# genlm/genlm-backend

Measured on AMD Instinct MI355X. Metric: particles/sec + logprob-kernel HBM GB/s (% of 8 TB/s), 1024 particles gpt2, higher is better.
Workload: dtype f32

## Files before the change

### genlm-backend_amd/_lib.py

```python
import ctypes as C
import os

_HERE = os.path.dirname(os.path.abspath(__file__))
LIB_PATH = os.path.join(_HERE, "libglb_hip.so")

ABI_VERSION = 9
GLB_OK, GLB_EINVAL, GLB_EUNSUPPORTED, GLB_EHIP, GLB_ENOSPC = 0, 1, 2, 3, 4
F32, BF16, F16 = 0, 1, 2
MASK_NONE, MASK_BITS, MASK_F32, MASK_PREPARED = 0, 1, 2, 3
RNG_NONE, RNG_PHILOX, RNG_NOISE = 0, 1, 2
STEP_HW_EXP = 1
GEMM_BIAS, GEMM_BIAS_GELU_TANH = 0, 1
GEMM_FORM_LARGE, GEMM_FORM_SMALL = 1, 2


class GlbError(RuntimeError):
    def __init__(self, code, msg):
        super().__init__(f"glb error {code}: {msg}")
        self.code = code


class StepArgs(C.Structure):
    _fields_ = [
        ("struct_size", C.c_uint32),
# ... 139 lines not shown
    _fields_ = [
        ("struct_size", C.c_uint32),
        ("window", C.c_void_p), ("window_out", C.c_void_p), ("polys", C.c_void_p),
        ("n_small", C.c_int32), ("n_big", C.c_int32),
        ("vocab", C.c_int64), ("max_draw_rows", C.c_int64),
        ("n_draw", C.c_void_p),
        ("n_out_rows", C.c_int64),
        ("row_slot", C.c_void_p),
        ("out", C.c_void_p), ("out_ld", C.c_int64),
        ("workspace", C.c_void_p), ("workspace_bytes", C.c_size_t),
        ("reuse_windows", C.c_int32), ("rows_from", C.c_void_p), ("rows_from_ld", C.c_int64),
    ]


class GemmArgs(C.Structure):
    _fields_ = [
        ("struct_size", C.c_uint32),
        ("m", C.c_int64), ("n", C.c_int64), ("k", C.c_int64),
        ("a", C.c_void_p), ("lda", C.c_int64),
        ("w_split", C.c_void_p),
        ("bias", C.c_void_p),
        ("c", C.c_void_p), ("ldc", C.c_int64),
        ("epilogue", C.c_int32),
    ]


class LoraJob(C.Structure):
    _fields_ = [
        ("struct_size", C.c_uint32),
        ("w_dtype", C.c_int32), ("ab_dtype", C.c_int32), ("w_transposed", C.c_int32),
        ("n_out", C.c_int64), ("k_in", C.c_int64), ("r", C.c_int64),
        ("w", C.c_void_p), ("ldw", C.c_int64),
        ("a", C.c_void_p), ("lda", C.c_int64),
        ("b", C.c_void_p), ("ldb", C.c_int64),
        ("scale", C.c_float),
        ("out", C.c_void_p), ("ldo", C.c_int64),
    ]


class LoraRowsEntry(C.Structure):
    _fields_ = [
        ("struct_size", C.c_uint32),
        ("ab_dtype", C.c_int32),
        ("n_out", C.c_int64), ("k_in", C.c_int64), ("r", C.c_int64),
        ("a", C.c_void_p), ("lda", C.c_int64),
        ("b", C.c_void_p), ("ldb", C.c_int64),
# ... 338 lines not shown
                                  _vp]),
    "glb_trie_workspace_ex": (_sz, [_i64, _i64]),
    "glb_trie_masses": (C.c_int, [C.POINTER(TrieArgs), _vp]),
    "glb_trie_rows_workspace": (_sz, [_i64, C.POINTER(TriePlan)]),
    "glb_trie_rows": (C.c_int, [C.POINTER(TrieRowsArgs), C.POINTER(TriePlan), _vp]),
    "glb_resample_workspace": (_sz, [_i64]),
    "glb_resample_systematic": (C.c_int, [_vp, _i64, C.c_uint64, C.c_uint64, _vp, _vp, _vp, _sz, _vp]),
    "glb_mt19937_seed": (None, [C.POINTER(MT19937), C.c_uint64]),
    "glb_mt19937_exponential_f32": (C.c_int, [C.POINTER(MT19937), _vp, _i64]),
    "glb_mt19937_window": (C.c_int, [C.c_uint64, _vp]),
    "glb_mt19937_jump_polys": (C.c_int, [_i64, _i32, _i32, _vp]),
    "glb_mt19937_jump_host": (C.c_int, [_vp, _vp, _vp]),
    "glb_mt19937_rows_workspace": (_sz, [_i64, _i32]),
    "glb_mt19937_exponential_rows": (C.c_int, [C.POINTER(MtRowsArgs), _vp]),
    "glb_comm_unique_id": (C.c_int, [_vp]),
    "glb_comm_init": (C.c_int, [_vp, _i32, _i32, C.POINTER(C.c_void_p)]),
    "glb_allgather_f32": (C.c_int, [_vp, _vp, _i64, _vp, _vp]),
    "glb_comm_destroy": (C.c_int, [_vp]),
    "glb_gemm_split_bytes": (_sz, [_i64, _i64]),
    "glb_gemm_split_weights": (C.c_int, [_vp, _i64, _i64, _i64, _vp, _sz, _vp]),
    "glb_gemm_f32_split": (C.c_int, [C.POINTER(GemmArgs), _vp]),
    "glb_gemm_split_pick": (C.c_int, [_i64, _i64, _i64, C.c_int, C.POINTER(C.c_int)]),
    "glb_gemm_f32_split_form": (C.c_int, [C.POINTER(GemmArgs), C.c_int, _vp]),
    "glb_gemm_split_blocks_per_cu": (C.c_int, [C.c_int, C.POINTER(C.c_int)]),
    "glb_gemm_split_form_blocks_per_cu": (C.c_int, [C.c_int, C.c_int, C.POINTER(C.c_int)]),
    "glb_lora_merge_workspace_bytes": (_sz, [_i32]),
    "glb_lora_merge": (C.c_int, [C.POINTER(LoraJob), _i32, _vp, _sz, _vp]),
    "glb_lora_rows_table_bytes": (_sz, [_i32, _i32]),
    "glb_lora_rows_table_upload": (C.c_int, [C.POINTER(LoraRowsEntry), _i32, _i32, _vp, _sz, _vp]),
    "glb_lora_rows_workspace_bytes": (_sz, [_i64, _i32]),
    "glb_lora_rows": (C.c_int, [C.POINTER(LoraRowsArgs), _vp]),
    "glb_w4_bytes": (_sz, [_i64, _i64]),
    "glb_w4_quantize": (C.c_int, [C.POINTER(W4Args), _vp]),
    "glb_w4_dequantize": (C.c_int, [C.POINTER(W4Args), _vp]),
    "glb_w4_gemm_max_rows": (C.c_int, []),
    "glb_w4_gemm_workspace_bytes": (_sz, [_i64, _i64, _i64]),
    "glb_w4_gemm": (C.c_int, [C.POINTER(W4GemmArgs), _vp]),
    "glb_dfa_bank_init": (C.c_int, [C.POINTER(DfaArgs), _vp]),
    "glb_dfa_advance": (C.c_int, [C.POINTER(DfaArgs), _vp]),
    "glb_dfa_claim_rows": (C.c_int, [C.POINTER(DfaArgs), _vp]),
    "glb_dfa_fill_masks": (C.c_int, [C.POINTER(DfaArgs), _vp]),
    "glb_dfa_mask_ids": (C.c_int, [C.POINTER(DfaArgs), _vp]),
    "glb_dfa_bank_rows": (_i64, [_sz, _i64, _i64]),
    "glb_dfa_weight_bank_init": (C.c_int, [C.POINTER(DfaWeightArgs), _vp]),
    "glb_dfa_fill_weights": (C.c_int, [C.POINTER(DfaWeightArgs), _vp]),
    "glb_dfa_weight_bank_rows": (_i64, [_sz, _i64, _i64]),
# ... 64 lines not shown
```

### genlm-backend_amd/csrc/glb_gemm.hip

```cpp
#include <hip/hip_runtime.h>

#include <cstdint>

#include "../../include/glb.h"
#include "glb_common.hpp"

namespace {

typedef __attribute__((ext_vector_type(2))) float f32x2;
typedef __attribute__((ext_vector_type(4))) float f32x4;
typedef __attribute__((ext_vector_type(2))) __bf16 bf16x2;
typedef __attribute__((ext_vector_type(8))) __bf16 bf16x8;
typedef __attribute__((ext_vector_type(4))) uint32_t u32x4;

constexpr int BK = 32, THREADS = 256, WAVES = THREADS / 64;
constexpr int PIECE = 1024;

template <int MF_, int NF_, int BLOCKS_>
struct Geom {
  static constexpr int MF = MF_, NF = NF_, BLOCKS_PER_CU = BLOCKS_;
  static constexpr int BM = WAVES * MF * 16, BN = NF * 16;
  static constexpr int B_PIECES = NF * 3;
  static constexpr int WAVE_PIECES = B_PIECES / WAVES;
  static constexpr int STAGE_BYTES = B_PIECES * PIECE;
  static constexpr int LDS_BYTES = 2 * STAGE_BYTES;
// ... 39 lines not shown
  const int64_t t = (int64_t)blockIdx.x * blockDim.x + threadIdx.x;
  if (t >= (n / 16) * kb_count * 64) return;
  const int l = (int)(t & 63);
  const int64_t blk = t >> 6, kb = blk % kb_count, nb = blk / kb_count;
  const int64_t col = nb * 16 + (l & 15), row = kb * BK + 8 * (l >> 4);
  f32x4 x0, x1;
#pragma unroll
  for (int j = 0; j < 4; ++j) {
    x0[j] = w[(row + j) * ldw + col];
    x1[j] = w[(row + 4 + j) * ldw + col];
  }
  bf16x8 h, m, lo;
  split8(x0, x1, h, m, lo);
  u32x4 *dst = out + blk * 3 * 64 + l;
  dst[0] = __builtin_bit_cast(u32x4, h);
  dst[64] = __builtin_bit_cast(u32x4, m);
  dst[128] = __builtin_bit_cast(u32x4, lo);
}

__device__ __forceinline__ void glds16(const void *src, char *lds) {
  __builtin_amdgcn_global_load_lds(src, (__attribute__((address_space(3))) void *)lds, 16, 0, 0);
}

template <class G, bool GELU>
__global__ __launch_bounds__(THREADS, G::BLOCKS_PER_CU) void gemm_split_kernel(const float *__restrict__ a, int64_t lda,
                                                                const char *__restrict__ wsplit, const float *__restrict__ bias,
                                                                float *__restrict__ c, int64_t ldc, int m, int n, int k) {
  constexpr int MF = G::MF, NF = G::NF, BM = G::BM, BN = G::BN, WAVE_PIECES = G::WAVE_PIECES, STAGE_BYTES = G::STAGE_BYTES;
  extern __shared__ __attribute__((aligned(16))) char lds[];
  const int tid = threadIdx.x, lane = tid & 63, wave = tid >> 6;
  const int ntn = n / BN, ntm = (m + BM - 1) / BM;
  const int nwg = ntm * ntn, orig = blockIdx.x, xcd = orig & 7, q = nwg >> 3, r = nwg & 7;
  const int wgid = (xcd < r ? xcd * (q + 1) : r * (q + 1) + (xcd - r) * q) + (orig >> 3);
  const int tm = wgid / ntn, tn = wgid % ntn;
  const int m0 = tm * BM, n0 = tn * BN;
  const int kt_count = k / BK;

  const float *a_src[MF];
#pragma unroll
  for (int i = 0; i < MF; ++i) {
    int row = m0 + (MF * wave + i) * 16 + (lane & 15);
    row = row < m ? row : m - 1;
    a_src[i] = a + (int64_t)row * lda + 8 * (lane >> 4);
  }
  const char *b_src[WAVE_PIECES];
  int b_dst[WAVE_PIECES];
#pragma unroll
  for (int i = 0; i < WAVE_PIECES; ++i) {
    const int p = WAVE_PIECES * wave + i, nf = p / 3, pl = p % 3;
    const int64_t nb = n0 / 16 + nf;
// ... 41 lines not shown
      load_a(kt + 1);
      stage_b(cur ^ 1, kt + 1);
    }
#pragma unroll
    for (int nf = 0; nf < NF; ++nf) {
      const bf16x8 bh = *(const bf16x8 *)(base + (0 * NF + nf) * PIECE + lane * 16);
      const bf16x8 bm = *(const bf16x8 *)(base + (1 * NF + nf) * PIECE + lane * 16);
      const bf16x8 bl = *(const bf16x8 *)(base + (2 * NF + nf) * PIECE + lane * 16);
#pragma unroll
      for (int i = 0; i < MF; ++i) {
        f32x4 t = __builtin_amdgcn_mfma_f32_16x16x32_bf16(am[i], bm, f32x4{0.f, 0.f, 0.f, 0.f}, 0, 0, 0);
        t = __builtin_amdgcn_mfma_f32_16x16x32_bf16(al[i], bh, t, 0, 0, 0);
        t = __builtin_amdgcn_mfma_f32_16x16x32_bf16(ah[i], bl, t, 0, 0, 0);
        t = __builtin_amdgcn_mfma_f32_16x16x32_bf16(am[i], bh, t, 0, 0, 0);
        t = __builtin_amdgcn_mfma_f32_16x16x32_bf16(ah[i], bm, t, 0, 0, 0);
        t = __builtin_amdgcn_mfma_f32_16x16x32_bf16(ah[i], bh, t, 0, 0, 0);
        acc[i][nf] += t;
      }
    }
    asm volatile("s_waitcnt vmcnt(0)" ::: "memory");
    __syncthreads();
  }

#pragma unroll
  for (int nf = 0; nf < NF; ++nf) {
    const int col = n0 + nf * 16 + (lane & 15);
    const float b = bcol[nf];
#pragma unroll
    for (int i = 0; i < MF; ++i) {
      const int row0 = m0 + wave * (MF * 16) + i * 16 + 4 * (lane >> 4);
#pragma unroll
      for (int j = 0; j < 4; ++j) {
        const int row = row0 + j;
        if (row < m) {
          float v = acc[i][nf][j] + b;
          if (GELU) v = gelu_tanh(v);
          c[(int64_t)row * ldc + col] = v;
        }
      }
    }
  }
}

bool shape_supported(int64_t k, int64_t n) { return k > 0 && n > 0 && n % BN_MAX == 0 && k % 64 == 0 && k <= (1 << 20) && n <= (1 << 20); }

template <class G, bool GELU>
struct Form {
  static inline std::atomic<uint64_t> lds_done{0};
  static const void *kernel() { return (const void *)gemm_split_kernel<G, GELU>; }
  static int launch(const glb_gemm_args &g, hipStream_t stream) {
    const int64_t tiles = ((g.m + G::BM - 1) / G::BM) * (g.n / G::BN);
    if (tiles > INT32_MAX / 2 || g.m > INT32_MAX / 2) return glb::api_fail(GLB_EUNSUPPORTED, "too many rows");
    hipError_t e = glb::allow_dynamic_lds(kernel(), G::LDS_BYTES, lds_done);
    if (e != hipSuccess) return glb::api_hip_fail(e, "split GEMM LDS attribute");
    hipLaunchKernelGGL((gemm_split_kernel<G, GELU>), dim3((unsigned)tiles), dim3(THREADS), G::LDS_BYTES, stream, g.a, g.lda,
                       (const char *)g.w_split, g.bias, g.c, g.ldc, (int)g.m, (int)g.n, (int)g.k);
    e = hipGetLastError();
    if (e != hipSuccess) return glb::api_hip_fail(e, "split GEMM launch");
    return GLB_OK;
  }
  static int blocks_per_cu(int *blocks) {
    hipError_t e = glb::allow_dynamic_lds(kernel(), G::LDS_BYTES, lds_done);
    if (e != hipSuccess) return glb::api_hip_fail(e, "split GEMM LDS attribute");
    e = hipOccupancyMaxActiveBlocksPerMultiprocessor(blocks, gemm_split_kernel<G, GELU>, THREADS, G::LDS_BYTES);
    if (e != hipSuccess) return glb::api_hip_fail(e, "split GEMM occupancy query");
    return GLB_OK;
  }
};

bool form_ok(int form) { return form == GLB_GEMM_FORM_LARGE || form == GLB_GEMM_FORM_SMALL; }

hipError_t device_cus(int *n_cus) {
  static std::atomic<int> cached[64];
  int dev = 0;
  hipError_t e = hipGetDevice(&dev);
  if (e != hipSuccess) return e;
  const bool slot = dev >= 0 && dev < 64;
  if (slot && (*n_cus = cached[dev].load(std::memory_order_relaxed)) > 0) return hipSuccess;
  e = hipDeviceGetAttribute(n_cus, hipDeviceAttributeMultiprocessorCount, dev);
  if (e == hipSuccess && slot) cached[dev].store(*n_cus, std::memory_order_relaxed);
  return e;
}

constexpr int PICK_TILES_NUM = 3, PICK_TILES_DEN = 2;

}

// ... 10 lines not shown
  if (!shape_supported(k, n)) return glb::api_fail(GLB_EUNSUPPORTED, "split GEMM needs n %% 128 == 0 and k %% 64 == 0");
  if (out_bytes < glb_gemm_split_bytes(k, n) || ((uintptr_t)out) % 16)
    return glb::api_fail(GLB_ENOSPC, "split weight buffer too small or not 16-byte aligned");
  const int64_t threads = (n / 16) * (k / BK) * 64;
  hipLaunchKernelGGL(split_weights_kernel, dim3(blocks_for(threads, 256)), dim3(256), 0, (hipStream_t)stream, w, k, n, ldw,
                     (u32x4 *)out);
  const hipError_t e = hipGetLastError();
  if (e != hipSuccess) return glb::api_hip_fail(e, "split_weights launch");
  return GLB_OK;
}


int glb_gemm_split_pick(int64_t m, int64_t n, int64_t k, int n_cus, int *form) {
  if (!form) return glb::api_fail(GLB_EINVAL, "null pointer");
  if (m <= 0 || n <= 0 || k <= 0 || n_cus <= 0)
    return glb::api_fail(GLB_EINVAL, "bad shape (m %lld, n %lld, k %lld, %d CUs)", (long long)m, (long long)n, (long long)k,
                         n_cus);
  if (m > INT32_MAX || n > INT32_MAX) return *form = GLB_GEMM_FORM_LARGE, GLB_OK;
  const int64_t tiles = ((m + Large::BM - 1) / Large::BM) * ((n + Large::BN - 1) / Large::BN);
  *form = tiles * PICK_TILES_DEN < (int64_t)PICK_TILES_NUM * n_cus ? GLB_GEMM_FORM_SMALL : GLB_GEMM_FORM_LARGE;
  return GLB_OK;
}

int glb_gemm_f32_split_form(const glb_gemm_args *args, int form, void *stream) {
  if (!args) return glb::api_fail(GLB_EINVAL, "null argument block");
  if (args->struct_size != sizeof(glb_gemm_args))
    return glb::api_fail(GLB_EINVAL, "glb_gemm_args.struct_size %u != %zu (ABI mismatch)", args->struct_size,
                         sizeof(glb_gemm_args));
  if (form != 0 && !form_ok(form)) return glb::api_fail(GLB_EINVAL, "bad form %d", form);
  const glb_gemm_args &g = *args;
  if (!g.a || !g.w_split || !g.c) return glb::api_fail(GLB_EINVAL, "null pointer");
  if (g.m <= 0 || g.n <= 0 || g.k <= 0 || g.lda < g.k || g.ldc < g.n)
    return glb::api_fail(GLB_EINVAL, "bad shape (m %lld, n %lld, k %lld, lda %lld, ldc %lld)", (long long)g.m,
                         (long long)g.n, (long long)g.k, (long long)g.lda, (long long)g.ldc);
  if (g.epilogue != GLB_GEMM_BIAS && g.epilogue != GLB_GEMM_BIAS_GELU_TANH)
    return glb::api_fail(GLB_EINVAL, "bad epilogue %d", g.epilogue);
  if (!shape_supported(g.k, g.n)) return glb::api_fail(GLB_EUNSUPPORTED, "split GEMM needs n %% 128 == 0 and k %% 64 == 0");
  if (((uintptr_t)g.a) % 16 || g.lda % 4 || ((uintptr_t)g.w_split) % 16)
    return glb::api_fail(GLB_EUNSUPPORTED, "split GEMM needs A and its row pitch 16-byte aligned");
  if (form == 0) {
    int n_cus = 0;
    const hipError_t e = device_cus(&n_cus);
    if (e != hipSuccess) return glb::api_hip_fail(e, "split GEMM CU count");
    const int rc = glb_gemm_split_pick(g.m, g.n, g.k, n_cus, &form);
    if (rc != GLB_OK) return rc;
  }
  const bool gelu = g.epilogue == GLB_GEMM_BIAS_GELU_TANH;
  hipStream_t s = (hipStream_t)stream;
  if (form == GLB_GEMM_FORM_SMALL) return gelu ? Form<Small, true>::launch(g, s) : Form<Small, false>::launch(g, s);
  return gelu ? Form<Large, true>::launch(g, s) : Form<Large, false>::launch(g, s);
}

int glb_gemm_f32_split(const glb_gemm_args *args, void *stream) { return glb_gemm_f32_split_form(args, 0, stream); }

int glb_gemm_split_form_blocks_per_cu(int form, int gelu, int *blocks) {
  if (!blocks) return glb::api_fail(GLB_EINVAL, "null pointer");
  if (!form_ok(form)) return glb::api_fail(GLB_EINVAL, "bad form %d", form);
  if (form == GLB_GEMM_FORM_SMALL) return gelu ? Form<Small, true>::blocks_per_cu(blocks) : Form<Small, false>::blocks_per_cu(blocks);
  return gelu ? Form<Large, true>::blocks_per_cu(blocks) : Form<Large, false>::blocks_per_cu(blocks);
}

int glb_gemm_split_blocks_per_cu(int gelu, int *blocks) {
  return glb_gemm_split_form_blocks_per_cu(GLB_GEMM_FORM_LARGE, gelu, blocks);
}

}
```

### genlm-backend_amd/engine.py

```python
import ctypes as C

import numpy as np
import torch

from . import _lib
from ._lib import GLB_EHIP, GlbError
from ._lib import (F32, BF16, F16, MASK_NONE, MASK_BITS, MASK_F32, MASK_PREPARED, RNG_NONE, RNG_PHILOX, RNG_NOISE,
                   STEP_HW_EXP, KvPlanArgs, KvPlanChunkArgs, MtRowsArgs, StepArgs, TrieArgs, TriePlan, TrieRowsArgs, MT19937, MT_POLY_WORDS, check)

_DT = {torch.float32: F32, torch.bfloat16: BF16, torch.float16: F16}


def _ptr(t):
    return None if t is None else C.c_void_p(t.data_ptr())


class LoraRowsTable:

    def __init__(self, dev, n_slots, n_modules, r_max, keep):
        self.dev, self.n_slots, self.n_modules, self.r_max, self.keep = dev, n_slots, n_modules, r_max, keep


class HostRng:

# ... 725 lines not shown
                check(self.lib.glb_gemm_split_blocks_per_cu(int(bool(gelu)), C.byref(blocks)))
            else:
                check(self.lib.glb_gemm_split_form_blocks_per_cu(int(form), int(bool(gelu)), C.byref(blocks)))
        return blocks.value

    def gemm_split_pick(self, m, n, k, n_cus=None):
        if n_cus is None:
            n_cus = torch.cuda.get_device_properties(self.device).multi_processor_count
        form = C.c_int(0)
        check(self.lib.glb_gemm_split_pick(m, n, k, n_cus, C.byref(form)))
        return form.value

    def gemm_split_weights(self, w):
        k, n = w.shape
        nbytes = self.lib.glb_gemm_split_bytes(k, n)
        if nbytes == 0 or w.dtype != torch.float32 or w.stride(1) != 1:
            return None
        if w.device != self.device:
            raise ValueError(f"tensor on {w.device}, engine on {self.device}")
        out =torch.empty(nbytes, dtype=torch.uint8, device=self.device)
        check(self.lib.glb_gemm_split_weights(_ptr(w), k, n, w.stride(0), _ptr(out), nbytes, self._stream()))
        return out

    def gemm_split(self, x, w_split, n, bias=None, gelu=False, out=None, form=None):
        k = x.shape[-1]
        x2 = x.reshape(-1, k)
        m = x2.shape[0]
        if m == 0 or x2.stride(1) != 1:
            return None
        if bias is not None:
            if bias.device != self.device:
                raise ValueError(f"bias on {bias.device}, engine on {self.device}")
            if bias.dim() != 1 or bias.numel() != n:
                raise ValueError(f"bias of shape {tuple(bias.shape)}, expected ({n},)")
            if bias.dtype != torch.float32 or bias.stride(0) != 1:
                return None
        if out is None:
            out = torch.empty((m, n), dtype=torch.float32, device=self.device)
        else:
            if out.device != self.device:
                raise ValueError(f"out on {out.device}, engine on {self.device}")
            if out.dtype != torch.float32 or tuple(out.shape) != (m, n):
                raise ValueError(f"out is {out.dtype} {tuple(out.shape)}, expected torch.float32 {(m, n)}")
            if out.stride(1) != 1 or (m > 1 and out.stride(0) < n):
                raise ValueError(f"out has strides {out.stride()}: rows of unit inner stride, at least {n} apart, are needed")
        a = _lib.GemmArgs()
        a.struct_size = C.sizeof(_lib.GemmArgs)
        a.m, a.n, a.k = m, n, k
        a.a, a.lda = x2.data_ptr(), x2.stride(0)
        a.w_split = w_split.data_ptr()
        a.bias = bias.data_ptr() if bias is not None else None
        a.c, a.ldc = out.data_ptr(), max(out.stride(0), n)
        a.epilogue = _lib.GEMM_BIAS_GELU_TANH if gelu else _lib.GEMM_BIAS
        if form is None:
            rc = self.lib.glb_gemm_f32_split(C.byref(a), self._stream())
        else:
            rc = self.lib.glb_gemm_f32_split_form(C.byref(a), int(form), self._stream())
        if rc == _lib.GLB_EUNSUPPORTED:
            return None
        check(rc)
        return out.view(*x.shape[:-1], n)

    def lora_merge(self, jobs):
        n = len(jobs)
        if n == 0:
            return
        table = (_lib.LoraJob * n)()
        for q, j in zip(table, jobs):
            w, a, b, out = j["w"], j["a"], j["b"], j["out"]
            for t in (w, a, b, out):
                if t.device != self.device:
                    raise ValueError(f"tensor on {t.device}, engine on {self.device}")
                if t.dim() != 2 or t.stride(1) != 1:
                    raise ValueError("lora_merge: every matrix must be 2-D with unit inner stride")
                if t.dtype not in _DT:
                    raise ValueError(f"lora_merge: unsupported dtype {t.dtype}")
            if a.dtype != b.dtype or out.dtype != w.dtype or out.shape != w.shape:
                raise ValueError("lora_merge: a / b must share a dtype, out must match w's dtype and shape")
            tr = bool(j.get("transposed", False))
            q.struct_size = C.sizeof(_lib.LoraJob)
            q.w_dtype, q.ab_dtype, q.w_transposed = _DT[w.dtype], _DT[a.dtype], int(tr)
            q.k_in, q.n_out = (w.shape[0], w.shape[1]) if tr else (w.shape[1], w.shape[0])
            q.r = a.shape[0]
            if tuple(a.shape) != (q.r, q.k_in) or tuple(b.shape) != (q.n_out, q.r):
# ... 537 lines not shown
```

### genlm-backend_amd/fuse.py

```python
import copy
import types

import torch

RMSNORM_CLASSES = ("LlamaRMSNorm", "MistralRMSNorm", "Qwen2RMSNorm", "Qwen3RMSNorm")
ROPE_ATTENTION_CLASSES = ("LlamaAttention",)


def shadow_model(model):
    cfg = getattr(model, "config", None)
    new_cfg = copy.copy(cfg) if cfg is not None else None
    memo = {}

    def walk(mod):
        got = memo.get(id(mod))
        if got is not None:
            return got
        new = copy.copy(mod)
        memo[id(mod)] = new
        new._modules = {name: (walk(child) if child is not None else None) for name, child in mod._modules.items()}
        if cfg is not None and new.__dict__.get("config") is cfg:
            new.__dict__["config"] = new_cfg
        return new

# ... 79 lines not shown
        self.engine = engine

    def __enter__(self):
        self.was = getattr(self.engine, "_split_all_rows", False)
        self.engine._split_all_rows = True
        return self

    def __exit__(self, *exc):
        self.engine._split_all_rows = self.was
        return False


def _is_tanh_gelu(act):
    return isinstance(act, torch.nn.GELU) and act.approximate == "tanh"


class SplitConv1D(torch.nn.Module):

    def __init__(self, src, engine, min_rows):
        super().__init__()
        self._parameters = src._parameters
        self.nf, self.nx = src.nf, src.nx
        self.min_rows = min_rows
        self.__dict__["_glb_engine"] = engine

    def _split(self):
        w = self.weight
        key = (id(w), w._version, w.data_ptr())
        ent = self.__dict__.get("_glb_split")
        if ent is None or ent[0] != key:
            with torch.no_grad():
                img = self._glb_engine.gemm_split_weights(w)
            ent = self.__dict__["_glb_split"] = (key, img, w)
        return ent[1]

    def _native(self, x):
        w = self.weight
        return (x.dtype == torch.float32 and w.dtype == torch.float32 and x.is_cuda and x.device == w.device
                and x.device == self._glb_engine.device
                and (x.shape[:-1].numel() >= self.min_rows or getattr(self._glb_engine, "_split_all_rows", False))
                and not (torch.is_grad_enabled() and (x.requires_grad or w.requires_grad
                                                      or (self.bias is not None and self.bias.requires_grad))))

    def forward(self, x, act=None):
        if self._native(x):
            img = self._split()
            if img is not None:
                gelu = _is_tanh_gelu(act)
                y = self._glb_engine.gemm_split(x, img, self.nf, self.bias, gelu=gelu)
                if y is not None:
                    return y if gelu or act is None else act(y)
        size_out = x.size()[:-1] + (self.nf,)
        y = torch.addmm(self.bias, x.view(-1, x.size(-1)), self.weight).view(size_out)
        return y if act is None else act(y)

    def extra_repr(self):
        return f"nf={self.nf}, nx={self.nx}, split-bf16 GEMM from {self.min_rows} rows"


def _gpt2_mlp_forward(self, hidden_states):
    h = self.c_fc(hidden_states, act=self.act)
    return self.dropout(self.c_proj(h))


def weights_version(net):
    v = 0
    for mod in net.modules():
        ent = mod.__dict__.get("_glb_qkv")
        if ent is not None and hasattr(mod.q_proj, "weight"):
            for t in (mod.q_proj.weight, mod.k_proj.weight, mod.v_proj.weight):
                v += t._version + (id(t) & 0xFFFF)
        if mod.__dict__.get("_glb_split") is not None:
            t = mod.weight
            v += t._version + (id(t) & 0xFFFF)
    return v


def _llama_attention_forward(self, hidden_states, position_embeddings=None, attention_mask=None, past_key_values=None,
                             **kwargs):
    from transformers.modeling_utils import ALL_ATTENTION_FUNCTIONS
    from transformers.models.llama.modeling_llama import eager_attention_forward

    w4 = not hasattr(self.q_proj, "weight")
    if torch.is_grad_enabled() and (hidden_states.requires_grad or (not w4 and self.q_proj.weight.requires_grad)):
        return type(self).forward(self, hidden_states, position_embeddings=position_embeddings, attention_mask=attention_mask,
# ... 59 lines not shown
                child.forward = types.MethodType(_llama_attention_forward, child)
                done.append("rope")
            elif kind == "LlamaRotaryEmbedding":
                child.forward = types.MethodType(_rotary_forward_signed, child)
            elif kind == "LlamaMLP" and merge_mlp:
                child.forward = types.MethodType(_llama_mlp_forward, child)
                done.append("gate_up")
    return done


def _split_conv1d(shadow, engine):
    done = []
    for mod in list(shadow.modules()):
        for name, child in list(mod._modules.items()):
            if type(child).__name__ != "Conv1D" or child.weight.dtype != torch.float32:
                continue
            min_rows = SPLIT_GEMM_MIN_ROWS.get((child.nf, child.nx))
            if min_rows is None or not engine.gemm_split_supports(child.nx, child.nf):
                continue
            mod._modules[name] = SplitConv1D(child, engine, min_rows)
            done.append("split_gemm")
        if type(mod).__name__ == "GPT2MLP" and isinstance(mod._modules.get("c_fc"), SplitConv1D):
            mod.forward = types.MethodType(_gpt2_mlp_forward, mod)
    return done
```

### genlm-backend_amd/kv.py

```python
import gc
import itertools
from collections import OrderedDict

import numpy as np
import torch
from transformers.cache_utils import Cache, CacheLayerMixin, DynamicCache


_ATTN_NAME = "glb"
SHORT_ATTENTION_MAX = 4096


def _glb_attention_forward(module, query, key, value, attention_mask, dropout=0.0, scaling=None, **kwargs):
    from transformers.integrations.sdpa_attention import sdpa_attention_forward

    layer = getattr(key, "_glb_layer", None)
    if layer is not None and layer._new_k is not None and getattr(layer.owner, "n_new", None) is not None:
        if key is not layer.keys or value is not layer.values:
            raise RuntimeError("glb_slab_attention_chunk: the attention module changed the key / value tensors the KV slab "
                               "handed out: the new tokens were never appended")
        k_new, v_new, layer._new_k, layer._new_v = layer._new_k, layer._new_v, None, None
        o = layer.owner
        scale = scaling if scaling is not None else query.shape[-1] ** -0.5
        return o.engine.slab_attention_chunk(query, k_new, v_new, layer.keys, layer.values, o.pos, o.n_new, scale, rows=o.rows), None
# ... 576 lines not shown
        layer = _PackedLayer(self)
        super().__init__(layers=[layer] * n_layers)


class PackedEncoding:

    def __init__(self, out, last, n_rows):
        self.out, self.hidden, self.last, self.n_rows = out, out.last_hidden_state[0], last, n_rows

    def last_rows(self):
        return self.hidden[self.last]


def packed_supported(llm):
    body, eng = llm._body, llm.engine
    cfg = getattr(body, "config", None)
    if cfg is None or getattr(cfg, "_attn_implementation", None) != _ATTN_NAME or getattr(cfg, "_glb_engine", None) is not eng:
        return False
    heads = getattr(cfg, "num_attention_heads", None)
    head_dim = getattr(cfg, "head_dim", None) or (cfg.hidden_size // heads if heads else None)
    return bool(head_dim in (16, 32, 64, 128) and getattr(cfg, "num_hidden_layers", 0) > 0)


def encode_packed(llm, batch, sel, n_sel, grp, groups, n_tail_rows, max_keys=PACKED_MAX_KEYS):
    eng, dev = llm.engine, llm.device
    tokens, starts, lengths = batch
    if not 1 <= max_keys <= PACKED_MAX_KEYS:
        raise ValueError(f"encode_packed serves contexts of up to {PACKED_MAX_KEYS} tokens")
    if n_sel < 1 or n_tail_rows < n_sel:
        raise ValueError("encode_packed: every context feeds at least one tail row")
    if not packed_supported(llm):
        raise RuntimeError("encode_packed: this model's attention is not served by glb_short_attention")
    G, n_pre = len(groups.lens), groups.n_rows
    M = n_pre + int(n_tail_rows)
    sel_l, grp_l = sel[:n_sel].long(), grp[:n_sel].long().clamp(0, G - 1)
    pre_len, pre_start = groups.lens_d[grp_l], groups.starts_d[grp_l]
    tail = lengths[sel_l] - pre_len
    ends = torch.cumsum(tail, 0, dtype=torch.int32)
    tail_start = n_pre + ends - tail
    segments = torch.cat([groups.segments, torch.stack([pre_start, pre_len, tail_start, tail], 1)]).contiguous()
    r = torch.arange(int(n_tail_rows), dtype=torch.int32, device=dev)
    u = torch.searchsorted(ends, r, right=True).clamp_(max=n_sel - 1)
    pos_t = (pre_len[u] + (r - (ends - tail)[u])).long()
    at = (starts[sel_l[u]] + pos_t).clamp_(0, tokens.numel() - 1)
    ids = torch.cat([groups.ids, tokens[at].long()]).view(1, M)
    max_pos = getattr(llm._body.config, "max_position_embeddings", None) or (1 << 30)
    pos = torch.cat([groups.pos, pos_t.clamp_(0, min(PACKED_MAX_KEYS, max_pos) - 1)]).view(1, M)
    pkv = PackedKV(eng, segments, M, max_keys, llm._body.config.num_hidden_layers)
    out = llm._body(input_ids=ids, position_ids=pos, attention_mask=None, past_key_values=pkv, use_cache=True)
    if pkv.served != len(pkv.layers):
        raise RuntimeError(f"glb_short_attention_packed served {pkv.served} of {len(pkv.layers)} layers: an attention module "
                           "bypassed the attention interface and attended across the packed contexts")
    return PackedEncoding(out, (tail_start + tail - 1).long().clamp_(0, M - 1), M)


class PrefixLRU:

    def __init__(self, budget_bytes, on_remove=None):
        self.budget = int(budget_bytes)
        self.used = 0
        self._od = OrderedDict()
        self.evictions = 0
        self.on_remove = on_remove

    def put(self, node, kv):
        self.drop(node)
        size = kv.nbytes()
        node.past_key_values = kv
        self._od[id(node)] = (node, size)
        self.used += size
        while self.used > self.budget and len(self._od) > 1:
            _, (old, sz) = self._od.popitem(last=False)
            old.past_key_values = None
            self.used -= sz
            self.evictions += 1
            if self.on_remove is not None:
# ... 31 lines not shown
```

### include/glb.h

```cpp
#ifndef GLB_H
#define GLB_H

#include <stddef.h>
#include <stdint.h>

#ifdef __cplusplus
extern "C" {
#endif

#define GLB_ABI_VERSION 9

enum {
  GLB_OK = 0,
  GLB_EINVAL = 1,
  GLB_EUNSUPPORTED = 2,
  GLB_EHIP = 3,
  GLB_ENOSPC = 4
};

enum { GLB_F32 = 0, GLB_BF16 = 1, GLB_F16 = 2 };

enum {
  GLB_MASK_NONE = 0,
  GLB_MASK_BITS = 1,
// ... 277 lines not shown
int glb_comm_unique_id(void *out_id);
int glb_comm_init(const void *id, int32_t rank, int32_t world, void **out_comm);
int glb_allgather_f32(void *comm, const float *send, int64_t n, float *recv, void *hip_stream);
int glb_comm_destroy(void *comm);

enum { GLB_GEMM_BIAS = 0, GLB_GEMM_BIAS_GELU_TANH = 1 };
typedef struct glb_gemm_args {
  uint32_t struct_size;
  int64_t m, n, k;
  const float *a;
  int64_t lda;
  const void *w_split;
  const float *bias;
  float *c;
  int64_t ldc;
  int32_t epilogue;
} glb_gemm_args;
size_t glb_gemm_split_bytes(int64_t k, int64_t n);
int glb_gemm_split_weights(const float *w, int64_t k, int64_t n, int64_t ldw, void *out, size_t out_bytes, void *hip_stream);
int glb_gemm_f32_split(const glb_gemm_args *args, void *hip_stream);
enum { GLB_GEMM_FORM_LARGE = 1, GLB_GEMM_FORM_SMALL = 2 };
int glb_gemm_split_pick(int64_t m, int64_t n, int64_t k, int n_cus, int *form);
int glb_gemm_f32_split_form(const glb_gemm_args *args, int form, void *hip_stream);
int glb_gemm_split_blocks_per_cu(int gelu, int *blocks);
int glb_gemm_split_form_blocks_per_cu(int form, int gelu, int *blocks);

typedef struct glb_lora_job {
  uint32_t struct_size;
  int32_t w_dtype;
  int32_t ab_dtype;
  int32_t w_transposed;
  int64_t n_out, k_in, r;
  const void *w;
  int64_t ldw;
  const void *a;
  int64_t lda;
  const void *b;
  int64_t ldb;
  float scale;
  void *out;
  int64_t ldo;
} glb_lora_job;
size_t glb_lora_merge_workspace_bytes(int32_t n_jobs);
int glb_lora_merge(const glb_lora_job *jobs , int32_t n_jobs, void *workspace , size_t workspace_bytes,
                   void *hip_stream);

typedef struct glb_lora_rows_entry {
  uint32_t struct_size;
// ... 418 lines not shown
```

Before: 142,600.

## Fuse residual add into split GEMM epilogue and build packed plan natively

Adds a residual-add epilogue to the split f32 GEMM and patches GPT-2 blocks to offer the residual to the attention and MLP c_proj layers, so the separate elementwise add kernel and its extra read/write of the hidden states are dropped. Also adds a native two-kernel packed-plan builder (a scan plus per-row gather) to replace the chain of small torch ops (cumsum, searchsorted, gathers, cat) used to build packed encoding inputs. Risks include a single-block scan kernel for large selections and extra epilogue register pressure from preloading residual values.

```diff
diff --git a/genlm-backend_amd/_lib.py b/genlm-backend_amd/_lib.py
--- a/genlm-backend_amd/_lib.py
+++ b/genlm-backend_amd/_lib.py
@@ -185,6 +185,18 @@
         ("bias", C.c_void_p),
         ("c", C.c_void_p), ("ldc", C.c_int64),
         ("epilogue", C.c_int32),
+    ]
+
+
+class PackedPlanArgs(C.Structure):
+    _fields_ = [
+        ("struct_size", C.c_uint32),
+        ("n_tokens", C.c_int64), ("n_contexts", C.c_int64), ("n_sel", C.c_int64), ("n_groups", C.c_int64),
+        ("n_pre", C.c_int64), ("n_tail_rows", C.c_int64), ("pos_cap", C.c_int64),
+        ("tokens", C.c_void_p), ("starts", C.c_void_p), ("lengths", C.c_void_p), ("sel", C.c_void_p), ("grp", C.c_void_p),
+        ("group_starts", C.c_void_p), ("group_lens", C.c_void_p), ("group_segments", C.c_void_p),
+        ("group_ids", C.c_void_p), ("group_pos", C.c_void_p),
+        ("segments", C.c_void_p), ("ids", C.c_void_p), ("pos", C.c_void_p), ("last", C.c_void_p), ("ends", C.c_void_p),
     ]
 
 
@@ -569,6 +581,8 @@
     "glb_gemm_f32_split": (C.c_int, [C.POINTER(GemmArgs), _vp]),
     "glb_gemm_split_pick": (C.c_int, [_i64, _i64, _i64, C.c_int, C.POINTER(C.c_int)]),
     "glb_gemm_f32_split_form": (C.c_int, [C.POINTER(GemmArgs), C.c_int, _vp]),
+    "glb_gemm_f32_split_residual": (C.c_int, [C.POINTER(GemmArgs), _vp, _i64, C.c_int, _vp]),
+    "glb_packed_plan": (C.c_int, [C.POINTER(PackedPlanArgs), _vp]),
     "glb_gemm_split_blocks_per_cu": (C.c_int, [C.c_int, C.POINTER(C.c_int)]),
     "glb_gemm_split_form_blocks_per_cu": (C.c_int, [C.c_int, C.c_int, C.POINTER(C.c_int)]),
     "glb_lora_merge_workspace_bytes": (_sz, [_i32]),
diff --git a/genlm-backend_amd/csrc/glb_gemm.hip b/genlm-backend_amd/csrc/glb_gemm.hip
--- a/genlm-backend_amd/csrc/glb_gemm.hip
+++ b/genlm-backend_amd/csrc/glb_gemm.hip
@@ -1,6 +1,7 @@
 #include <hip/hip_runtime.h>
 
 #include <cstdint>
+#include <type_traits>
 
 #include "../../include/glb.h"
 #include "glb_common.hpp"
@@ -86,10 +87,21 @@
   __builtin_amdgcn_global_load_lds(src, (__attribute__((address_space(3))) void *)lds, 16, 0, 0);
 }
 
-template <class G, bool GELU>
-__global__ __launch_bounds__(THREADS, G::BLOCKS_PER_CU) void gemm_split_kernel(const float *__restrict__ a, int64_t lda,
-                                                                const char *__restrict__ wsplit, const float *__restrict__ bias,
-                                                                float *__restrict__ c, int64_t ldc, int m, int n, int k) {
+enum Epi { EPI_NONE, EPI_GELU, EPI_RESIDUAL };
+
+template <bool ON>
+struct Residual {
+  const float *p;
+  int64_t ld;
+};
+template <>
+struct Residual<false> {};
+
+template <class G, Epi EPI>
+__global__ __launch_bounds__(THREADS, G::BLOCKS_PER_CU) void gemm_split_kernel(
+    const float *__restrict__ a, int64_t lda, const char *__restrict__ wsplit, const float *__restrict__ bias,
+    typename std::conditional<EPI == EPI_RESIDUAL, float *, float *__restrict__>::type c, int64_t ldc, int m, int n, int k,
+    Residual<EPI == EPI_RESIDUAL> res) {
   constexpr int MF = G::MF, NF = G::NF, BM = G::BM, BN = G::BN, WAVE_PIECES = G::WAVE_PIECES, STAGE_BYTES = G::STAGE_BYTES;
   extern __shared__ __attribute__((aligned(16))) char lds[];
   const int tid = threadIdx.x, lane = tid & 63, wave = tid >> 6;
@@ -177,6 +189,19 @@
     __syncthreads();
   }
 
+  float rv[EPI == EPI_RESIDUAL ? MF : 1][EPI == EPI_RESIDUAL ? NF : 1][4];
+  if constexpr (EPI == EPI_RESIDUAL) {
+#pragma unroll
+    for (int nf = 0; nf < NF; ++nf)
+#pragma unroll
+      for (int i = 0; i < MF; ++i)
+#pragma unroll
+        for (int j = 0; j < 4; ++j) {
+          const int row = m0 + wave * (MF * 16) + i * 16 + 4 * (lane >> 4) + j;
+          rv[i][nf][j] = row < m ? res.p[(int64_t)row * res.ld + n0 + nf * 16 + (lane & 15)] : 0.0f;
+        }
+  }
+
 #pragma unroll
   for (int nf = 0; nf < NF; ++nf) {
     const int col = n0 + nf * 16 + (lane & 15);
@@ -189,7 +214,8 @@
         const int row = row0 + j;
         if (row < m) {
           float v = acc[i][nf][j] + b;
-          if (GELU) v = gelu_tanh(v);
+          if (EPI == EPI_GELU) v = gelu_tanh(v);
+          if (EPI == EPI_RESIDUAL) v += rv[i][nf][j];
           c[(int64_t)row * ldc + col] = v;
         }
       }
@@ -199,17 +225,17 @@
 
 bool shape_supported(int64_t k, int64_t n) { return k > 0 && n > 0 && n % BN_MAX == 0 && k % 64 == 0 && k <= (1 << 20) && n <= (1 << 20); }
 
-template <class G, bool GELU>
+template <class G, Epi EPI>
 struct Form {
   static inline std::atomic<uint64_t> lds_done{0};
-  static const void *kernel() { return (const void *)gemm_split_kernel<G, GELU>; }
-  static int launch(const glb_gemm_args &g, hipStream_t stream) {
+  static const void *kernel() { return (const void *)gemm_split_kernel<G, EPI>; }
+  static int launch(const glb_gemm_args &g, hipStream_t stream, Residual<EPI == EPI_RESIDUAL> res = {}) {
     const int64_t tiles = ((g.m + G::BM - 1) / G::BM) * (g.n / G::BN);
     if (tiles > INT32_MAX / 2 || g.m > INT32_MAX / 2) return glb::api_fail(GLB_EUNSUPPORTED, "too many rows");
     hipError_t e = glb::allow_dynamic_lds(kernel(), G::LDS_BYTES, lds_done);
     if (e != hipSuccess) return glb::api_hip_fail(e, "split GEMM LDS attribute");
-    hipLaunchKernelGGL((gemm_split_kernel<G, GELU>), dim3((unsigned)tiles), dim3(THREADS), G::LDS_BYTES, stream, g.a, g.lda,
-                       (const char *)g.w_split, g.bias, g.c, g.ldc, (int)g.m, (int)g.n, (int)g.k);
+    hipLaunchKernelGGL((gemm_split_kernel<G, EPI>), dim3((unsigned)tiles), dim3(THREADS), G::LDS_BYTES, stream, g.a, g.lda,
+                       (const char *)g.w_split, g.bias, g.c, g.ldc, (int)g.m, (int)g.n, (int)g.k, res);
     e = hipGetLastError();
     if (e != hipSuccess) return glb::api_hip_fail(e, "split GEMM launch");
     return GLB_OK;
@@ -217,7 +243,7 @@
   static int blocks_per_cu(int *blocks) {
     hipError_t e = glb::allow_dynamic_lds(kernel(), G::LDS_BYTES, lds_done);
     if (e != hipSuccess) return glb::api_hip_fail(e, "split GEMM LDS attribute");
-    e = hipOccupancyMaxActiveBlocksPerMultiprocessor(blocks, gemm_split_kernel<G, GELU>, THREADS, G::LDS_BYTES);
+    e = hipOccupancyMaxActiveBlocksPerMultiprocessor(blocks, gemm_split_kernel<G, EPI>, THREADS, G::LDS_BYTES);
     if (e != hipSuccess) return glb::api_hip_fail(e, "split GEMM occupancy query");
     return GLB_OK;
   }
@@ -274,7 +300,7 @@
   return GLB_OK;
 }
 
-int glb_gemm_f32_split_form(const glb_gemm_args *args, int form, void *stream) {
+static int split_check(const glb_gemm_args *args, int &form) {
   if (!args) return glb::api_fail(GLB_EINVAL, "null argument block");
   if (args->struct_size != sizeof(glb_gemm_args))
     return glb::api_fail(GLB_EINVAL, "glb_gemm_args.struct_size %u != %zu (ABI mismatch)", args->struct_size,
@@ -297,10 +323,45 @@
     const int rc = glb_gemm_split_pick(g.m, g.n, g.k, n_cus, &form);
     if (rc != GLB_OK) return rc;
   }
+  return GLB_OK;
+}
+
+int glb_gemm_f32_split_form(const glb_gemm_args *args, int form, void *stream) {
+  const int rc = split_check(args, form);
+  if (rc != GLB_OK) return rc;
+  const glb_gemm_args &g = *args;
   const bool gelu = g.epilogue == GLB_GEMM_BIAS_GELU_TANH;
   hipStream_t s = (hipStream_t)stream;
-  if (form == GLB_GEMM_FORM_SMALL) return gelu ? Form<Small, true>::launch(g, s) : Form<Small, false>::launch(g, s);
-  return gelu ? Form<Large, true>::launch(g, s) : Form<Large, false>::launch(g, s);
+  if (form == GLB_GEMM_FORM_SMALL) return gelu ? Form<Small, EPI_GELU>::launch(g, s) : Form<Small, EPI_NONE>::launch(g, s);
+  return gelu ? Form<Large, EPI_GELU>::launch(g, s) : Form<Large, EPI_NONE>::launch(g, s);
+}
+
+int glb_gemm_f32_split_residual(const glb_gemm_args *args, const float *residual, int64_t ldr, int form, void *stream) {
+  const int rc = split_check(args, form);
+  if (rc != GLB_OK) return rc;
+  const glb_gemm_args &g = *args;
+  if (g.epilogue != GLB_GEMM_BIAS) return glb::api_fail(GLB_EINVAL, "the residual epilogue takes GLB_GEMM_BIAS only (epilogue %d)", g.epilogue);
+  if (!residual) return glb::api_fail(GLB_EINVAL, "null residual");
+  if (ldr < g.n || ((uintptr_t)residual) % sizeof(float))
+    return glb::api_fail(GLB_EINVAL, "residual misaligned or its pitch %lld below n %lld", (long long)ldr, (long long)g.n);
+  if (!(residual == g.c && ldr == g.ldc)) {
+    const uintptr_t c0 = (uintptr_t)g.c, c1 = c0 + ((uint64_t)(g.m - 1) * (uint64_t)g.ldc + (uint64_t)g.n) * sizeof(float);
+    const uintptr_t r0 = (uintptr_t)residual, r1 = r0 + ((uint64_t)(g.m - 1) * (uint64_t)ldr + (uint64_t)g.n) * sizeof(float);
+    if (r0 < c1 && c0 < r1) return glb::api_fail(GLB_EINVAL, "the residual overlaps C without being C");
+  }
+  int dev = 0;
+  hipError_t e = hipGetDevice(&dev);
+  if (e != hipSuccess) return glb::api_hip_fail(e, "split GEMM device");
+  hipPointerAttribute_t at;
+  e = hipPointerGetAttributes(&at, residual);
+  if (e != hipSuccess || at.type != hipMemoryTypeDevice || at.device != dev) {
+    (void)hipGetLastError();
+    return glb::api_fail(GLB_EINVAL, "the residual is not memory of the current device");
+  }
+  hipStream_t s = (hipStream_t)stream;
+  const Residual<true> res{residual, ldr};
+  if (form == GLB_GEMM_FORM_SMALL) return Form<Small, EPI_RESIDUAL>::launch(g, s, res);
+  return Form<Large, EPI_RESIDUAL>::launch(g, s, res);
 }
 
 int glb_gemm_f32_split(const glb_gemm_args *args, void *stream) { return glb_gemm_f32_split_form(args, 0, stream); }
@@ -308,8 +369,8 @@
 int glb_gemm_split_form_blocks_per_cu(int form, int gelu, int *blocks) {
   if (!blocks) return glb::api_fail(GLB_EINVAL, "null pointer");
   if (!form_ok(form)) return glb::api_fail(GLB_EINVAL, "bad form %d", form);
-  if (form == GLB_GEMM_FORM_SMALL) return gelu ? Form<Small, true>::blocks_per_cu(blocks) : Form<Small, false>::blocks_per_cu(blocks);
-  return gelu ? Form<Large, true>::blocks_per_cu(blocks) : Form<Large, false>::blocks_per_cu(blocks);
+  if (form == GLB_GEMM_FORM_SMALL) return gelu ? Form<Small, EPI_GELU>::blocks_per_cu(blocks) : Form<Small, EPI_NONE>::blocks_per_cu(blocks);
+  return gelu ? Form<Large, EPI_GELU>::blocks_per_cu(blocks) : Form<Large, EPI_NONE>::blocks_per_cu(blocks);
 }
 
 int glb_gemm_split_blocks_per_cu(int gelu, int *blocks) {
diff --git a/genlm-backend_amd/csrc/glb_packed_plan.hip b/genlm-backend_amd/csrc/glb_packed_plan.hip
--- /dev/null
+++ b/genlm-backend_amd/csrc/glb_packed_plan.hip
@@ -0,0 +1,116 @@
+#include <hip/hip_runtime.h>
+
+#include <cstdint>
+
+#include "../../include/glb.h"
+#include "glb_common.hpp"
+
+namespace {
+
+constexpr int SCAN_THREADS = 1024, ROW_THREADS = 256;
+
+__device__ __forceinline__ int32_t wrap_add(int32_t a, int32_t b) { return (int32_t)((uint32_t)a + (uint32_t)b); }
+__device__ __forceinline__ int32_t wrap_sub(int32_t a, int32_t b) { return (int32_t)((uint32_t)a - (uint32_t)b); }
+
+__device__ __forceinline__ int64_t ctx_index(int32_t s, int64_t n) {
+  int64_t i = s < 0 ? (int64_t)s + n : (int64_t)s;
+  return i < 0 ? 0 : (i >= n ? n - 1 : i);
+}
+
+__global__ __launch_bounds__(SCAN_THREADS) void packed_plan_scan_kernel(glb_packed_plan_args a) {
+  __shared__ int32_t wave_sum[SCAN_THREADS / 64];
+  __shared__ int32_t carry_s;
+  const int tid = threadIdx.x, lane = tid & 63, wave = tid >> 6;
+  const int64_t G = a.n_groups, U = a.n_sel;
+  for (int64_t i = tid; i < G * 4; i += SCAN_THREADS) a.segments[i] = a.group_segments[i];
+  if (tid == 0) carry_s = 0;
+  __syncthreads();
+  for (int64_t base = 0; base < U; base += SCAN_THREADS) {
+    const int64_t u = base + tid;
+    int32_t pre_len = 0, pre_start = 0, tail = 0;
+    if (u < U) {
+      int64_t g = a.grp[u];
+      g = g < 0 ? 0 : (g > G - 1 ? G - 1 : g);
+      pre_len = a.group_lens[g];
+      pre_start = a.group_starts[g];
+      tail = wrap_sub(a.lengths[ctx_index(a.sel[u], a.n_contexts)], pre_len);
+    }
+    int32_t x = tail;
+#pragma unroll
+    for (int d = 1; d < 64; d <<= 1) {
+      const int32_t y = __shfl_up(x, d, 64);
+      if (lane >= d) x = wrap_add(x, y);
+    }
+    if (lane == 63) wave_sum[wave] = x;
+    __syncthreads();
+    int32_t before = carry_s;
+    for (int w = 0; w < wave; ++w) before = wrap_add(before, wave_sum[w]);
+    const int32_t end = wrap_add(before, x);
+    if (u < U) {
+      const int32_t tail_start = wrap_sub(wrap_add((int32_t)a.n_pre, end), tail);
+      a.ends[u] = end;
+      int32_t *seg = a.segments + (G + u) * 4;
+      seg[0] = pre_start;
+      seg[1] = pre_len;
+      seg[2] = tail_start;
+      seg[3] = tail;
+      const int64_t last = (int64_t)wrap_sub(wrap_add(tail_start, tail), 1), m = a.n_pre + a.n_tail_rows;
+      a.last[u] = last < 0 ? 0 : (last > m - 1 ? m - 1 : last);
+    }
+    __syncthreads();
+    if (tid == SCAN_THREADS - 1) carry_s = end;
+    __syncthreads();
+  }
+}
+
+__global__ __launch_bounds__(ROW_THREADS) void packed_plan_rows_kernel(glb_packed_plan_args a) {
+  const int64_t row = (int64_t)blockIdx.x * ROW_THREADS + threadIdx.x;
+  if (row >= a.n_pre + a.n_tail_rows) return;
+  if (row < a.n_pre) {
+    a.ids[row] = a.group_ids[row];
+    a.pos[row] = a.group_pos[row];
+    return;
+  }
+  const int64_t U = a.n_sel;
+  const int32_t r = (int32_t)(row - a.n_pre);
+  int64_t lo = 0, hi = U;
+  while (lo < hi) {
+    const int64_t mid = lo + ((hi - lo) >> 1);
+    if (a.ends[mid] > r) hi = mid; else lo = mid + 1;
+  }
+  const int64_t u = lo > U - 1 ? U - 1 : lo;
+  const int32_t *seg = a.segments + (a.n_groups + u) * 4;
+  const int32_t pos_t = wrap_add(seg[1], wrap_sub(r, wrap_sub(a.ends[u], seg[3])));
+  int64_t at = a.starts[ctx_index(a.sel[u], a.n_contexts)] + (int64_t)pos_t;
+  at = at < 0 ? 0 : (at > a.n_tokens - 1 ? a.n_tokens - 1 : at);
+  a.ids[row] = (int64_t)a.tokens[at];
+  const int64_t p = pos_t;
+  a.pos[row] = p < 0 ? 0 : (p > a.pos_cap - 1 ? a.pos_cap - 1 : p);
+}
+
+}
+
+extern "C" int glb_packed_plan(const glb_packed_plan_args *args, void *stream) {
+  if (!args) return glb::api_fail(GLB_EINVAL, "glb_packed_plan: null argument block");
+  if (args->struct_size != sizeof(glb_packed_plan_args))
+    return glb::api_fail(GLB_EINVAL, "glb_packed_plan_args.struct_size %u != %zu (ABI mismatch)", args->struct_size,
+                         sizeof(glb_packed_plan_args));
+  const glb_packed_plan_args &a = *args;
+  if (a.n_groups < 1 || a.n_sel < 1 || a.n_pre < 1 || a.n_tail_rows < a.n_sel || a.n_contexts < 1 || a.n_tokens < 1 ||
+      a.pos_cap < 1 || a.n_sel > INT32_MAX || a.n_pre + a.n_tail_rows > INT32_MAX)
+    return glb::api_fail(GLB_EINVAL, "glb_packed_plan: bad sizes (G %lld, U %lld, prompt rows %lld, tail rows %lld, contexts %lld, "
+                         "tokens %lld, position cap %lld)", (long long)a.n_groups, (long long)a.n_sel, (long long)a.n_pre,
+                         (long long)a.n_tail_rows, (long long)a.n_contexts, (long long)a.n_tokens, (long long)a.pos_cap);
+  if (!a.tokens || !a.starts || !a.lengths || !a.sel || !a.grp || !a.group_starts || !a.group_lens || !a.group_segments ||
+      !a.group_ids || !a.group_pos)
+    return glb::api_fail(GLB_EINVAL, "glb_packed_plan: null input");
+  if (!a.segments || !a.ids || !a.pos || !a.last || !a.ends) return glb::api_fail(GLB_EINVAL, "glb_packed_plan: null output");
+  hipStream_t s = (hipStream_t)stream;
+  hipLaunchKernelGGL(packed_plan_scan_kernel, dim3(1), dim3(SCAN_THREADS), 0, s, a);
+  hipError_t e = hipGetLastError();
+  if (e != hipSuccess) return glb::api_hip_fail(e, "glb_packed_plan scan launch");
+  hipLaunchKernelGGL(packed_plan_rows_kernel, dim3(blocks_for(a.n_pre + a.n_tail_rows, ROW_THREADS)), dim3(ROW_THREADS), 0, s, a);
+  e = hipGetLastError();
+  if (e != hipSuccess) return glb::api_hip_fail(e, "glb_packed_plan rows launch");
+  return GLB_OK;
+}
diff --git a/genlm-backend_amd/engine.py b/genlm-backend_amd/engine.py
--- a/genlm-backend_amd/engine.py
+++ b/genlm-backend_amd/engine.py
@@ -771,7 +771,7 @@
         check(self.lib.glb_gemm_split_weights(_ptr(w), k, n, w.stride(0), _ptr(out), nbytes, self._stream()))
         return out
 
-    def gemm_split(self, x, w_split, n, bias=None, gelu=False, out=None, form=None):
+    def gemm_split(self, x, w_split, n, bias=None, gelu=False, out=None, form=None, residual=None):
         k = x.shape[-1]
         x2 = x.reshape(-1, k)
         m = x2.shape[0]
@@ -801,7 +801,18 @@
         a.bias = bias.data_ptr() if bias is not None else None
         a.c, a.ldc = out.data_ptr(), max(out.stride(0), n)
         a.epilogue = _lib.GEMM_BIAS_GELU_TANH if gelu else _lib.GEMM_BIAS
-        if form is None:
+        if residual is not None:
+            if gelu:
+                raise ValueError("gemm_split: the residual epilogue does not follow the GELU")
+            if residual.device != self.device:
+                raise ValueError(f"residual on {residual.device}, engine on {self.device}")
+            r2 = residual.view(-1, n) if residual.dim() != 2 else residual
+            if residual.dtype != torch.float32 or tuple(r2.shape) != (m, n) or r2.stride(1) != 1 or (m > 1 and r2.stride(0) < n):
+                raise ValueError(f"residual is {residual.dtype} {tuple(residual.shape)} with strides {residual.stride()}: "
+                                 f"torch.float32 {(m, n)} rows of unit inner stride are needed")
+            rc = self.lib.glb_gemm_f32_split_residual(C.byref(a), r2.data_ptr(), max(r2.stride(0), n), int(form or 0),
+                                                      self._stream())
+        elif form is None:
             rc = self.lib.glb_gemm_f32_split(C.byref(a), self._stream())
         else:
             rc = self.lib.glb_gemm_f32_split_form(C.byref(a), int(form), self._stream())
@@ -809,6 +820,33 @@
             return None
         check(rc)
         return out.view(*x.shape[:-1], n)
+
+    def packed_plan(self, batch, sel, n_sel, grp, groups, n_tail_rows, pos_cap):
+        tokens, starts, lengths = batch
+        G, n_pre = len(groups.lens), groups.n_rows
+        ins = (tokens, starts, lengths, sel, grp, groups.starts_d, groups.lens_d, groups.segments, groups.ids, groups.pos)
+        self._check_dev(*ins)
+        want = (torch.int32, torch.int64, torch.int32, torch.int32, torch.int32, torch.int32, torch.int32, torch.int32,
+                torch.int64, torch.int64)
+        if any(t.dtype != d for t, d in zip(ins, want)):
+            raise ValueError(f"packed_plan: dtypes {[t.dtype for t in ins]}, expected {list(want)}")
+        if sel.numel() < n_sel or grp.numel() < n_sel or starts.numel() != lengths.numel() or groups.ids.numel() != n_pre:
+            raise ValueError("packed_plan: sel / grp shorter than n_sel, or starts / lengths / the prompts' rows disagree")
+        M = n_pre + int(n_tail_rows)
+        seg = torch.empty((G + n_sel, 4), dtype=torch.int32, device=self.device)
+        ids = torch.empty(M, dtype=torch.int64, device=self.device)
+        pos = torch.empty(M, dtype=torch.int64, device=self.device)
+        last = torch.empty(n_sel, dtype=torch.int64, device=self.device)
+        ends = self._i32(n_sel)
+        a = _lib.PackedPlanArgs()
+        a.struct_size = C.sizeof(_lib.PackedPlanArgs)
+        a.n_tokens, a.n_contexts, a.n_sel, a.n_groups = tokens.numel(), lengths.numel(), n_sel, G
+        a.n_pre, a.n_tail_rows, a.pos_cap = n_pre, int(n_tail_rows), int(pos_cap)
+        (a.tokens, a.starts, a.lengths, a.sel, a.grp, a.group_starts, a.group_lens, a.group_segments, a.group_ids,
+         a.group_pos) = (t.data_ptr() for t in ins)
+        a.segments, a.ids, a.pos, a.last, a.ends = (t.data_ptr() for t in (seg, ids, pos, last, ends))
+        check(self.lib.glb_packed_plan(C.byref(a), self._stream()))
+        return seg, ids, pos, last
 
     def lora_merge(self, jobs):
         n = len(jobs)
diff --git a/genlm-backend_amd/fuse.py b/genlm-backend_amd/fuse.py
--- a/genlm-backend_amd/fuse.py
+++ b/genlm-backend_amd/fuse.py
@@ -125,6 +125,7 @@
         self._parameters = src._parameters
         self.nf, self.nx = src.nf, src.nx
         self.min_rows = min_rows
+        self.fused_residuals = 0
         self.__dict__["_glb_engine"] = engine
 
     def _split(self):
@@ -145,11 +146,27 @@
                 and not (torch.is_grad_enabled() and (x.requires_grad or w.requires_grad
                                                       or (self.bias is not None and self.bias.requires_grad))))
 
+    def offer_residual(self, residual):
+        self.__dict__["_glb_residual"] = residual
+
+    def residual_taken(self):
+        self.__dict__.pop("_glb_residual", None)
+        return self.__dict__.pop("_glb_residual_taken", False)
+
     def forward(self, x, act=None):
+        residual = self.__dict__.pop("_glb_residual", None)
         if self._native(x):
             img = self._split()
             if img is not None:
                 gelu = _is_tanh_gelu(act)
+                if (residual is not None and act is None and residual.dtype == torch.float32 and residual.device == x.device
+                        and residual.shape == x.shape[:-1] + (self.nf,) and residual.is_contiguous()
+                        and not (torch.is_grad_enabled() and residual.requires_grad)):
+                    y = self._glb_engine.gemm_split(x, img, self.nf, self.bias, residual=residual)
+                    if y is not None:
+                        self.__dict__["_glb_residual_taken"] = True
+                        self.fused_residuals += 1
+                        return y
                 y = self._glb_engine.gemm_split(x, img, self.nf, self.bias, gelu=gelu)
                 if y is not None:
                     return y if gelu or act is None else act(y)
@@ -164,6 +181,38 @@
 def _gpt2_mlp_forward(self, hidden_states):
     h = self.c_fc(hidden_states, act=self.act)
     return self.dropout(self.c_proj(h))
+
+
+RESIDUAL_EPILOGUE = True
+
+
+def _gpt2_block_forward(self, hidden_states, past_key_values=None, attention_mask=None, encoder_hidden_states=None,
+                        encoder_attention_mask=None, use_cache=False, **kwargs):
+    if encoder_hidden_states is not None or not RESIDUAL_EPILOGUE:
+        return type(self).forward(self, hidden_states, past_key_values=past_key_values, attention_mask=attention_mask,
+                                  encoder_hidden_states=encoder_hidden_states, encoder_attention_mask=encoder_attention_mask,
+                                  use_cache=use_cache, **kwargs)
+    residual = hidden_states
+    proj = self.attn._modules.get("c_proj")
+    offered = isinstance(proj, SplitConv1D) and not self.attn.training
+    if offered:
+        proj.offer_residual(residual)
+    try:
+        attn_output, _ = self.attn(self.ln_1(hidden_states), past_key_values=past_key_values, attention_mask=attention_mask,
+                                   use_cache=use_cache, **kwargs)
+    finally:
+        taken = offered and proj.residual_taken()
+    hidden_states = attn_output if taken else attn_output + residual
+    residual = hidden_states
+    proj = self.mlp._modules.get("c_proj")
+    offered = isinstance(proj, SplitConv1D) and not self.mlp.training
+    if offered:
+        proj.offer_residual(residual)
+    try:
+        feed_forward_hidden_states = self.mlp(self.ln_2(hidden_states))
+    finally:
+        taken = offered and proj.residual_taken()
+    return feed_forward_hidden_states if taken else residual + feed_forward_hidden_states
 
 
 def weights_version(net):
@@ -269,4 +318,8 @@
             done.append("split_gemm")
         if type(mod).__name__ == "GPT2MLP" and isinstance(mod._modules.get("c_fc"), SplitConv1D):
             mod.forward = types.MethodType(_gpt2_mlp_forward, mod)
+    for mod in shadow.modules():
+        if type(mod).__name__ == "GPT2Block" and any(
+                isinstance(getattr(mod, part)._modules.get("c_proj"), SplitConv1D) for part in ("attn", "mlp") if hasattr(mod, part)):
+            mod.forward = types.MethodType(_gpt2_block_forward, mod)
     return done
diff --git a/genlm-backend_amd/kv.py b/genlm-backend_amd/kv.py
--- a/genlm-backend_amd/kv.py
+++ b/genlm-backend_amd/kv.py
@@ -622,17 +622,16 @@
     return bool(head_dim in (16, 32, 64, 128) and getattr(cfg, "num_hidden_layers", 0) > 0)
 
 
-def encode_packed(llm, batch, sel, n_sel, grp, groups, n_tail_rows, max_keys=PACKED_MAX_KEYS):
+def _packed_plan_arrays(llm, batch, sel, n_sel, grp, groups, n_tail_rows, native_plan=True):
     eng, dev = llm.engine, llm.device
     tokens, starts, lengths = batch
-    if not 1 <= max_keys <= PACKED_MAX_KEYS:
-        raise ValueError(f"encode_packed serves contexts of up to {PACKED_MAX_KEYS} tokens")
-    if n_sel < 1 or n_tail_rows < n_sel:
-        raise ValueError("encode_packed: every context feeds at least one tail row")
-    if not packed_supported(llm):
-        raise RuntimeError("encode_packed: this model's attention is not served by glb_short_attention")
     G, n_pre = len(groups.lens), groups.n_rows
     M = n_pre + int(n_tail_rows)
+    max_pos = getattr(llm._body.config, "max_position_embeddings", None) or (1 << 30)
+    pos_cap = min(PACKED_MAX_KEYS, max_pos)
+    native = getattr(eng, "packed_plan", None) if native_plan else None
+    if native is not None:
+        return native(batch, sel, n_sel, grp, groups, n_tail_rows, pos_cap) + (M,)
     sel_l, grp_l = sel[:n_sel].long(), grp[:n_sel].long().clamp(0, G - 1)
     pre_len, pre_start = groups.lens_d[grp_l], groups.starts_d[grp_l]
     tail = lengths[sel_l] - pre_len
@@ -643,15 +642,27 @@
     u = torch.searchsorted(ends, r, right=True).clamp_(max=n_sel - 1)
     pos_t = (pre_len[u] + (r - (ends - tail)[u])).long()
     at = (starts[sel_l[u]] + pos_t).clamp_(0, tokens.numel() - 1)
-    ids = torch.cat([groups.ids, tokens[at].long()]).view(1, M)
-    max_pos = getattr(llm._body.config, "max_position_embeddings", None) or (1 << 30)
-    pos = torch.cat([groups.pos, pos_t.clamp_(0, min(PACKED_MAX_KEYS, max_pos) - 1)]).view(1, M)
+    ids = torch.cat([groups.ids, tokens[at].long()])
+    pos = torch.cat([groups.pos, pos_t.clamp_(0, pos_cap - 1)])
+    return segments, ids, pos, (tail_start + tail - 1).long().clamp_(0, M - 1), M
+
+
+def encode_packed(llm, batch, sel, n_sel, grp, groups, n_tail_rows, max_keys=PACKED_MAX_KEYS, native_plan=True):
+    eng = llm.engine
+    if not 1 <= max_keys <= PACKED_MAX_KEYS:
+        raise ValueError(f"encode_packed serves contexts of up to {PACKED_MAX_KEYS} tokens")
+    if n_sel < 1 or n_tail_rows < n_sel:
+        raise ValueError("encode_packed: every context feeds at least one tail row")
+    if not packed_supported(llm):
+        raise RuntimeError("encode_packed: this model's attention is not served by glb_short_attention")
+    segments, ids, pos, last, M = _packed_plan_arrays(llm, batch, sel, n_sel, grp, groups, n_tail_rows, native_plan)
+    ids, pos = ids.view(1, M), pos.view(1, M)
     pkv = PackedKV(eng, segments, M, max_keys, llm._body.config.num_hidden_layers)
     out = llm._body(input_ids=ids, position_ids=pos, attention_mask=None, past_key_values=pkv, use_cache=True)
     if pkv.served != len(pkv.layers):
         raise RuntimeError(f"glb_short_attention_packed served {pkv.served} of {len(pkv.layers)} layers: an attention module "
                            "bypassed the attention interface and attended across the packed contexts")
-    return PackedEncoding(out, (tail_start + tail - 1).long().clamp_(0, M - 1), M)
+    return PackedEncoding(out, last, M)
 
 
 class PrefixLRU:
diff --git a/include/glb.h b/include/glb.h
--- a/include/glb.h
+++ b/include/glb.h
@@ -323,8 +323,30 @@
 enum { GLB_GEMM_FORM_LARGE = 1, GLB_GEMM_FORM_SMALL = 2 };
 int glb_gemm_split_pick(int64_t m, int64_t n, int64_t k, int n_cus, int *form);
 int glb_gemm_f32_split_form(const glb_gemm_args *args, int form, void *hip_stream);
+int glb_gemm_f32_split_residual(const glb_gemm_args *args, const float *residual, int64_t ldr, int form, void *hip_stream);
 int glb_gemm_split_blocks_per_cu(int gelu, int *blocks);
 int glb_gemm_split_form_blocks_per_cu(int form, int gelu, int *blocks);
+
+typedef struct glb_packed_plan_args {
+  uint32_t struct_size;
+  int64_t n_tokens, n_contexts, n_sel, n_groups, n_pre, n_tail_rows, pos_cap;
+  const int32_t *tokens;
+  const int64_t *starts;
+  const int32_t *lengths;
+  const int32_t *sel;
+  const int32_t *grp;
+  const int32_t *group_starts;
+  const int32_t *group_lens;
+  const int32_t *group_segments;
+  const int64_t *group_ids;
+  const int64_t *group_pos;
+  int32_t *segments;
+  int64_t *ids;
+  int64_t *pos;
+  int64_t *last;
+  int32_t *ends;
+} glb_packed_plan_args;
+int glb_packed_plan(const glb_packed_plan_args *args, void *hip_stream);
 
 typedef struct glb_lora_job {
   uint32_t struct_size;
```

Result: faster. 149,400, median of 6 (+4.7%).
